# tangkk/audiomod

Hardware: AMD Instinct MI355X
Metric: Msamples/s (48 kHz stereo) phase-vocoder pitch-shift; x real-time per GPU (higher is better)
Workload: dtype f32; 1 GPU; configs[1]: normal_pitchshift +4 st, stereo 48 kHz, fft=2048, phase-locked; streams_per_gpu=128, channels=2, block=480, hop_in=203, slices_per_channel=14190, concurrent_stream_groups=1, parallelism=stream-sharded x1, no collective, rank_sync=none

## Files before the change

### audiomod_amd/csrc/pv_engine.cc

```cpp
#include <cstdio>
#include <cstdlib>
#include <cmath>
#include <algorithm>
#include <chrono>
#include <cstring>
#include <deque>
#include <memory>
#include <string>
#include <vector>

#include <hip/hip_runtime.h>

#include "audiomod_pv.h"
#include "pv_kernels.h"
#include "pv_wavefft.h"
#include "pv_plan.h"

namespace pv {

static thread_local std::string g_last_error;

static int hip_fail(hipError_t e, const char *what, int line) {
    char buf[512];
    snprintf(buf, sizeof buf, "%s failed at pv_engine.cc:%d: %s", what, line, hipGetErrorString(e));
// ... 208 lines not shown
    const ResTile *res_tiles;
    const uint2 *res_otab;
    int res_ntiles;
    hipStream_t res_stream;
    hipEvent_t ev_fused, ev_res, ev_ring_free;
    bool late_chain;
};

struct Core {
    Derived d;
    int device = 0, S = 0, C = 0, rows = 0;
    int Tc = 0, TR = 0, FR = 0, HP = 0, pkmax = 0, PKP = 0, lookback = 0;
    bool pipelined_planes = false;
    int ola_lds_floats = 0;
    int otab_off = 0, wacc_pitch = 0;
    DevTables tb{};
    DevBuf<int32_t> perm, iperm;
    DevBuf<float2> tw_fwd, tw_inv, st_fwd, st_inv;
    DevBuf<float4> twl_fwd, twl_inv;
    DevBuf<float> window, window_sh, sinc;
    DevBuf<float4> tab4;
    DevBuf<float> mag, phase, outphase, frames, rot;
    DevBuf<float> cmag, cphase;
    DevBuf<uint16_t> peaks;
    DevBuf<int32_t> npk, modes;
    DevBuf<PeakRec> recs;
    DevBuf<float> st_pp, st_po, st_rot;
    DevBuf<int32_t> st_kind;
    bool use_chain = false;
    bool chain_required = false;
    static constexpr int kChainMinRows = 192;
    bool fast_arith = false;
    bool fuse_phase = false;
    bool split_analysis = false;
    bool ahead = false;
    bool three_stage = false;
    int chain_AR = 0, chain_smask = 0, chain_waves = 0;
    int chain_max_adv = 0;
    DevBuf<float> st_acc, stream;
    mutable int acc_half = 0;
#ifdef PV_DIAG
    static bool debug_stale_acc() {
        static const bool on = [] {
            const char *e = getenv("AUDIOMOD_PV_DEBUG_STALE_ACC");
            return e && atoi(e) != 0;
        }();
        return on;
    }
#endif
    mutable hipError_t launch_err = hipSuccess;
    mutable int launch_err_line = 0;
    int take_launch_error() const {
        if (launch_err == hipSuccess) return PV_OK;
        const int rc = hip_fail(launch_err, "a launch / event call of Core::launch_chunk", launch_err_line);
        launch_err = hipSuccess;
        return rc;
    }
    void build_res_tiles(int64_t ka, int64_t kb, std::vector<ResTile> &tiles, std::vector<uint2> &otab) const;
    static bool chain_wanted() {
        const char *e = getenv("AUDIOMOD_PV_FUSED");
        if (e && atoi(e) == 0) return false;
        const char *sl = getenv("AUDIOMOD_PV_STREAM_LAUNCHES");
        return !(sl && strcmp(sl, "single") == 0);
    }
    bool wave_fft() const { return d.fft.nc == 256 || d.fft.nc == 512 || d.fft.nc == 1024 || d.fft.nc == 2048; }
    bool fast_chain() const { return use_chain && fast_capable(); }
// ... 134 lines not shown
    }
    TR = (nstreams > 0 && pipelined_planes) ? (ahead ? 3 : 2) * Tc + 1 : Tc + 1;
    FR = next_pow2_i(Tc + lookback + 1);

    std::vector<int32_t> ip(d.fft.nc);
    for (int j = 0; j < d.fft.nc; ++j) ip[d.fft.perm[j]] = j;
    if ((st = perm.upload(d.fft.perm)) != PV_OK) return st;
    if ((st = iperm.upload(ip)) != PV_OK) return st;
    auto up2 = [&](DevBuf<float2> &b, const std::vector<cpx> &v) -> int {
        std::vector<float2> t(v.size());
        for (size_t i = 0; i < v.size(); ++i) t[i] = make_float2(v[i].r, v[i].i);
        return b.upload(t);
    };
    if ((st = up2(tw_fwd, d.fft.tw_fwd)) != PV_OK) return st;
    if ((st = up2(tw_inv, d.fft.tw_inv)) != PV_OK) return st;
    if ((st = up2(st_fwd, d.fft.st_fwd)) != PV_OK) return st;
    if (wave_fft()) {
        auto lane_table = [&](const std::vector<cpx> &tw, DevBuf<float4> &dst) -> int {
            std::vector<cf> twc(tw.size());
            for (size_t i = 0; i < tw.size(); ++i) twc[i] = cf{tw[i].r, tw[i].i};
            const int entries = d.fft.nc == 256    ? wf_lane_table_entries<WF<256>>()
                                : d.fft.nc == 512  ? wf_lane_table_entries<WF<512>>()
                                : d.fft.nc == 1024 ? wf_lane_table_entries<WF<1024>>()
                                                   : wf_lane_table_entries<WF<2048>>();
            std::vector<cf> out(2 * (size_t)entries * 64);
            if (d.fft.nc == 256) wf_build_lane_table<WF<256>>(twc.data(), out.data());
            else if (d.fft.nc == 512) wf_build_lane_table<WF<512>>(twc.data(), out.data());
            else if (d.fft.nc == 1024) wf_build_lane_table<WF<1024>>(twc.data(), out.data());
            else wf_build_lane_table<WF<2048>>(twc.data(), out.data());
            std::vector<float4> o4((size_t)entries * 64);
            for (size_t i = 0; i < o4.size(); ++i) o4[i] = make_float4(out[2 * i].x, out[2 * i].y, out[2 * i + 1].x, out[2 * i + 1].y);
            return dst.upload(o4);
        };
        {
            const char *es = getenv("AUDIOMOD_PV_SPLIT_ANALYSIS");
            const char *sl = getenv("AUDIOMOD_PV_STREAM_LAUNCHES");
            split_analysis = d.fft.nc == 2048 && !(es && atoi(es) == 0) && !(sl && strcmp(sl, "single") == 0);
        }
        if (split_analysis) {
            std::vector<cf> twc(d.fft.tw_fwd.size());
            for (size_t i = 0; i < twc.size(); ++i) twc[i] = cf{d.fft.tw_fwd[i].r, d.fft.tw_fwd[i].i};
            const int entries = wf_lane_table_entries<WF2048S>();
            std::vector<cf> out(2 * (size_t)entries * WF2048S::LANES);
            wf_build_lane_table<WF2048S>(twc.data(), out.data());
            std::vector<float4> o4((size_t)entries * WF2048S::LANES);
            for (size_t i = 0; i < o4.size(); ++i) o4[i] = make_float4(out[2 * i].x, out[2 * i].y, out[2 * i + 1].x, out[2 * i + 1].y);
            if ((st = twl_fwd.upload(o4)) != PV_OK) return st;
        } else if ((st = lane_table(d.fft.tw_fwd, twl_fwd)) != PV_OK) return st;
        if ((st = lane_table(d.fft.tw_inv, twl_inv)) != PV_OK) return st;
    }
    if ((st = up2(st_inv, d.fft.st_inv)) != PV_OK) return st;
    if ((st = window.upload(d.window)) != PV_OK) return st;
    {
        const size_t pitch = (size_t)d.N + 8;
        std::vector<float> sh(4 * pitch, 0.f);
        for (int dd = 0; dd < 4; ++dd)
            for (int j = 0; j < d.N; ++j) sh[dd * pitch + j + dd] = d.window[j];
        if ((st = window_sh.upload(sh)) != PV_OK) return st;
    }
    if ((st = sinc.upload(d.sinc)) != PV_OK) return st;
    {
        std::vector<float4> t4;
        if (d.resample && d.interp) {
            t4.assign((size_t)d.oversample * (d.filt_len + 1), make_float4(0, 0, 0, 0));
            for (int off = 0; off < d.oversample; ++off)
                for (int j = 0; j < d.filt_len; ++j) {
// ... 231 lines not shown
    auto rec = [&](int i) {
        if (ev) HIPV(hipEventRecord(ev[i], st));
    };
    auto side_stream = [&](int k, auto &&launch_on) {
        if (defer_chain) return;
        if (part == 1) {
            HIPV(hipEventRecord(ev_match, st));
            HIPV(hipStreamWaitEvent(st_chain, ev_match, 0));
            if (ev) HIPV(hipEventRecord(ev[2 * k], st_chain));
            launch_on(st_chain);
            if (ev) HIPV(hipEventRecord(ev[2 * k + 1], st_chain));
            HIPV(hipEventRecord(ev_chain, st_chain));
        } else if (part == 2) {
            if (!only_resample) HIPV(hipStreamWaitEvent(st, ev_chain, 0));
        } else {
            rec(2 * k);
            launch_on(st);
            rec(2 * k + 1);
        }
    };
    AnalyzeArgs aa{};
    aa.tb = tb;
    aa.ia = ia;
    aa.hop = d.hop;
    const int s0 = (int)(t0 % TR);
    aa.t0 = t0;
    aa.s0 = s0;
    aa.Tn = Tn;
    aa.TR = TR;
    aa.rows = rows;
    aa.PKP = PKP;
    aa.find_peaks = cm == 1 ? 1 : 0;
    aa.split = split_analysis ? 1 : 0;
    aa.mag = mag.p;
    aa.phase = phase.p;
    aa.peaks = peaks.p;
    aa.npk = npk.p;
    const bool do_analysis = front && !only_chain && !no_analysis;
    if (do_analysis) rec(2 * PV_K_ANALYZE);
    if (single_launch) fused.aa = aa;
    else if (do_analysis) launch_analyze(aa, st); HIPV(hipGetLastError());
    if (do_analysis && d.vocoder && carrier) {
        AnalyzeArgs ca = aa;
        ca.ia = *carrier;
        ca.rows = 1;
        ca.find_peaks = 0;
        ca.mag = cmag.p;
        ca.phase = cphase.p;
        launch_analyze(ca, st); HIPV(hipGetLastError());
    }
    if (do_analysis) rec(2 * PV_K_ANALYZE + 1);
    if (only_analysis) return;

    if (cm == 1) {
        MatchArgs ma{};
        ma.N = d.N;
        ma.hs = d.hs;
        ma.HP = HP;
        ma.PKP = PKP;
        ma.C = C;
        ma.hop = d.hop;
        ma.TR = TR;
        ma.rows = rows;
        ma.Tn = Tn;
        ma.two_pi_hop = d.two_pi_hop;
        ma.t0 = t0;
// ... 2986 lines not shown
```

### audiomod_amd/csrc/pv_kernels.h

```cpp
#pragma once

#include <cstdint>

#include <hip/hip_runtime.h>

namespace pv {

constexpr int kFftThreads = 256;
constexpr int kTileOut = 256;
constexpr int kMaxTileFrames = 128;

struct DevTables {
    int N, hs, H, HP, nc, log2nc;
    int nstages;
    int radix[16], log2m[16], fstride[16];
    const int32_t *perm;
    const int32_t *iperm;
    const float2 *tw_fwd, *tw_inv, *st_fwd, *st_inv;
    const float4 *twl_fwd, *twl_inv;
    const float *window;
    const float *window_sh;
};

struct InAddr {
    const float *in;
    int64_t stride_s, stride_c;
    uint64_t mask;
    int64_t len;
};

enum : int { kModeInit = 0, kModeProp = 1, kModeLock = 2 };

struct AnalyzeArgs {
    DevTables tb;
    InAddr ia;
    int hop;
    int64_t t0;
    int s0;
    int Tn;
    int TR;
    int rows;
    int PKP;
    int find_peaks;
    int split;
    float *mag;
    float *phase;
    uint16_t *peaks;
    int32_t *npk;
};

struct PeakRec {
    float adv;
    float a2;
    float a1;
    uint32_t p1r1;
};

struct MatchArgs {
    int N, hs, HP, PKP, C, hop, TR, rows, Tn, s0;
    double two_pi_hop;
    int64_t t0;
    const int32_t *phase_inc;
    const float *phase;
    const uint16_t *peaks;
    const int32_t *npk;
    PeakRec *recs;
    int32_t *modes;
};

struct SeqArgs {
    int N, hs, HP, PKP, C, hop, TR, rows, Tn, s0;
    int high_prio;
    int narrow;
    double two_pi_hop;
    int64_t t0;
    const int32_t *phase_inc;
    const float *phase;
    const uint16_t *peaks;
    const int32_t *npk;
    const PeakRec *recs;
    const int32_t *modes;
// ... 254 lines not shown
```

### audiomod_amd/csrc/pv_kernels.hip

```cpp
#include "pv_kernels.h"
#include "pv_atan2f.h"
#include "pv_sincos.h"
#include "pv_wavefft.h"

#include <hip/hip_runtime.h>
#include <cstdlib>

namespace pv {

#ifdef PV_POISON
__device__ __forceinline__ void pv_poison_lds(char *base) {
    const uint32_t bytes = ((const __attribute__((address_space(4))) uint32_t *)__builtin_amdgcn_dispatch_ptr())[7];
    const int nt = blockDim.x * blockDim.y * blockDim.z, tid = threadIdx.x;
    for (uint32_t i = tid; i < bytes / 4; i += nt) reinterpret_cast<uint32_t *>(base)[i] = 0x7fc0dead;
    __syncthreads();
}
#define PV_POISON_LDS(base) pv_poison_lds(base)
#else
#define PV_POISON_LDS(base) ((void)0)
#endif

#define PV_PI 3.14159265358979323846

__device__ __forceinline__ float2 cmul(float2 a, float2 b) {
// ... 169 lines not shown

    const int lane = threadIdx.x & 63, wave = threadIdx.x >> 6, nw = nt >> 6;
    const int J = (hs + nt - 1) / nt;
    for (int j = 0; j < J; ++j) {
        const unsigned long long bm = __ballot(is_peak(smag, threadIdx.x + j * nt, hs));
        if (lane == 0) wcnt[j * nw + wave] = __popcll(bm);
    }
    __syncthreads();
    uint16_t *__restrict__ pk = a.peaks + plane * a.PKP;
    int running = 0, qi = 0;
    for (int j = 0; j < J; ++j) {
        const int mine = j * nw + wave;
        for (; qi < mine; ++qi) running += wcnt[qi];
        const int b = threadIdx.x + j * nt;
        const bool isp = is_peak(smag, b, hs);
        const unsigned long long bm = __ballot(isp);
        if (isp) pk[running + __popcll(bm & ((1ull << lane) - 1ull))] = (uint16_t)b;
    }
    if (threadIdx.x == 0) {
        int total = 0;
        for (int q = 0; q < J * nw; ++q) total += wcnt[q];
        a.npk[plane] = total;
    }
}

template <int WPB> __device__ __forceinline__ bool block_to_row_slice_w(int Tn, int rows, int &row, int &tl) {
    const int groups = (Tn + WPB - 1) / WPB;
    const int b = blockIdx.x, xcd = b & 7, q = b >> 3;
    row = xcd + 8 * (q / groups);
    tl = __builtin_amdgcn_readfirstlane(WPB * (q % groups) + (threadIdx.x >> 6));
    return row < rows && tl < Tn;
}

template <int NC, uint32_t ATAB>
__device__ __forceinline__ void analyze_wave_role(const AnalyzeArgs &a, const int row, const int tl, cf *lds) {
    typedef __attribute__((address_space(3))) uint32_t lds_u32;
    const unsigned char *atab = reinterpret_cast<const unsigned char *>((uintptr_t)ATAB);
    using W = WF<NC>;
    constexpr int N = 2 * NC, hs = NC, R = W::R;
    const int lane = threadIdx.x & 63;
    const uint32_t atab_word = pv_atan_blob_dev.w[lane];
    const DevTables &tb = a.tb;
    const int64_t t = a.t0 + tl;
    const int slot = ring_slot(a.s0, tl, a.TR);
    const int64_t a0 = t * (int64_t)a.hop;
    const float *__restrict__ in = a.ia.in + (int64_t)row * a.ia.stride_c;
    const float *__restrict__ w = tb.window;
    const cf *__restrict__ tw = reinterpret_cast<const cf *>(tb.tw_fwd);
    const cf *__restrict__ stw = reinterpret_cast<const cf *>(tb.st_fwd);
    const cf2 *__restrict__ twl = reinterpret_cast<const cf2 *>(tb.twl_fwd);

    WfTw<W> T0, T1, T2;
    wf_load_pass_tw<W, 0>(T0, lane, tw);
    cf v[R];
    {
        const int lp = wf_lane_part<W>(0, lane);
        const int lsrc = wf_src_of<W>(lp);
        const uint64_t m0 = (uint64_t)a0 & a.ia.mask;
        if (a0 + N + 4 <= a.ia.len && ((m0 + (uint64_t)(N + 3)) & a.ia.mask) == m0 + (uint64_t)(N + 3)) {
            const float *__restrict__ fp = in + m0;
            const uintptr_t fa = reinterpret_cast<uintptr_t>(fp);
            const int d = (int)((fa & 15u) >> 2);
            const float4 *__restrict__ xb = reinterpret_cast<const float4 *>(fa & ~(uintptr_t)15);
            const float4 *__restrict__ wb = reinterpret_cast<const float4 *>(tb.window_sh + (size_t)d * (N + 8));
            constexpr int Q = N / 256;
            float4 *stage4 = reinterpret_cast<float4 *>(lds);
            float4 xt = make_float4(0.f, 0.f, 0.f, 0.f), wt = xt;
            if (lane == 0) {
                xt = xb[64 * Q];
                wt = wb[64 * Q];
            }
            constexpr int QS = Q < 8 ? Q : 8;
#pragma unroll
            for (int q0 = 0; q0 < Q; q0 += QS) {
                float4 xq[QS], wq[QS];
#pragma unroll
                for (int q = 0; q < QS; ++q) {
                    xq[q] = xb[lane + 64 * (q0 + q)];
                    wq[q] = wb[lane + 64 * (q0 + q)];
                }
#pragma unroll
                for (int q = 0; q < QS; ++q)
                    stage4[lane + 64 * (q0 + q)] =
                        make_float4(xq[q].x * wq[q].x, xq[q].y * wq[q].y, xq[q].z * wq[q].z, xq[q].w * wq[q].w);
            }
            if (lane == 0) stage4[64 * Q] = make_float4(xt.x * wt.x, xt.y * wt.y, xt.z * wt.z, xt.w * wt.w);
            wave_sync();
            const float *stage = reinterpret_cast<const float *>(lds) + d;
            const int kl = (2 * lsrc + hs) & (N - 1);
#pragma unroll
            for (int r = 0; r < R; ++r) {
                const int kr = 2 * wf_src_of_const<W>(wf_reg_part<W>(0, r));
                const int k0 = kl ^ kr;
                v[r] = cf{stage[k0], stage[k0 + 1]};
            }
            wave_sync();
        } else {
#pragma unroll
            for (int r = 0; r < R; ++r) {
                const int src = lsrc | wf_src_of_const<W>(wf_reg_part<W>(0, r));
                const int k0 = (2 * src + hs) & (N - 1);
                const int64_t g0 = a0 + k0;
                const float x0 = g0 < a.ia.len ? in[(uint64_t)g0 & a.ia.mask] : 0.f;
                const float x1 = g0 + 1 < a.ia.len ? in[(uint64_t)(g0 + 1) & a.ia.mask] : 0.f;
                v[r] = cf{x0 * w[k0], x1 * w[k0 + 1]};
            }
        }
    }
    constexpr int J = NC / 128;
    const int lp0 = wf_lane_part<W>(0, lane), lp1 = wf_lane_part<W>(1, lane), lp2 = wf_lane_part<W>(2, lane);
    WfTwRaw<W, 1> raw1;
#if defined(PV_EXP_ANA) && (PV_EXP_ANA & 1)
#define PV_ANA_BFLY(x)
#else
#define PV_ANA_BFLY(x) x
#endif
#if defined(PV_EXP_ANA) && (PV_EXP_ANA & 2)
#define PV_ANA_XCHG(x)
#else
#define PV_ANA_XCHG(x) x
#endif
    wf_fetch_pass_tw<W, 1>(raw1, lane, twl);
    PV_ANA_BFLY((wf_apply_pass_stages<W, 0, false>(v, T0)));
    PV_ANA_XCHG((wf_store<W, 0>(lds, v, lp0)));
    wave_sync();
    PV_ANA_XCHG((wf_load<W, 1>(lds, v, lp1)));
    wf_unpack_pass_tw<W, 1>(T1, raw1);
    PV_ANA_BFLY((wf_apply_pass_stages<W, 1, false>(v, T1)));
    WfTwRaw<W, 2> raw2;
    wf_fetch_pass_tw<W, 2>(raw2, lane, twl);
    PV_ANA_XCHG((wf_store<W, 1>(lds, v, lp1)));
    wave_sync();
    PV_ANA_XCHG((wf_load<W, 2>(lds, v, lp2)));
    wf_unpack_pass_tw<W, 2>(T2, raw2);
    PV_ANA_BFLY((wf_apply_pass_stages<W, 2, false>(v, T2)));
    if constexpr (W::NPASS == 4) {
        const int lp3 = wf_lane_part<W>(3, lane);
        WfTwRaw<W, 3> raw3;
        wf_fetch_pass_tw<W, 3>(raw3, lane, twl);
        PV_ANA_XCHG((wf_store<W, 2>(lds, v, lp2)));
        wave_sync();
// ... 35 lines not shown
    if (lane == 0) {
        const cf fpk = lds[W::pad(NC / 2)];
        const cf fpnk = cf{fpk.x, -fpk.y};
        const cf f1k = wf_add(fpk, fpnk);
        const cf f2k = wf_sub(fpk, fpnk);
        const cf tq = wf_cmul(f2k, swmid);
        xmid = cf{(f1k.x - tq.x) * 0.5f, (tq.y - f1k.y) * 0.5f};
    }
    wave_sync();
#pragma unroll
    for (int j = 0; j < J; ++j) {
        const int k = lane + 64 * j;
        if (j == 0 && lane == 0) {
            lds[0] = xlo[0];
            lds[NC] = xhi[0];
        } else {
            lds[k] = xlo[j];
            lds[NC - k] = xhi[j];
        }
    }
    if (lane == 0) lds[NC / 2] = xmid;
    wave_sync();
    float *smag = reinterpret_cast<float *>(lds);
    *(lds_u32 *)(uintptr_t)(ATAB + 4u * (uint32_t)lane) = atab_word;
    float edge_mag = 0.f, edge_ph = 0.f;
    if (lane < 2) {
        const cf e = lds[lane == 0 ? 0 : NC];
        edge_mag = sqrtf(e.x * e.x + 0.f * 0.f);
        edge_ph = pv_u2f((uint32_t)((int32_t)pv_f2u(e.x) >> 31) & pv_f2u(3.1415927410e+00f));
    }
    wave_sync();
    if (lane == 0) lds[0] = cf{1.f, 1.f};
    wave_sync();
#pragma nounroll
    for (int q = 0; q < NC / 256; ++q) {
        const int i4 = 4 * (lane + 64 * q);
        const float4 c01 = *reinterpret_cast<const float4 *>(lds + i4);
        const float4 c23 = *reinterpret_cast<const float4 *>(lds + i4 + 2);
        float4 m4, p4;
        const float a0 = c01.x * c01.x + c01.y * c01.y, a1 = c01.z * c01.z + c01.w * c01.w;
        const float a2 = c23.x * c23.x + c23.y * c23.y, a3 = c23.z * c23.z + c23.w * c23.w;
        const float mx = __builtin_fmaxf(__builtin_fmaxf(pv_max3_abs(c01.x, c01.y, c01.z), pv_max3_abs(c01.w, c23.x, c23.y)),
                                         __builtin_fmaxf(__builtin_fabsf(c23.z), __builtin_fabsf(c23.w)));
        const float mn = __builtin_fminf(__builtin_fminf(pv_min3_abs(c01.x, c01.y, c01.z), pv_min3_abs(c01.w, c23.x, c23.y)),
                                         __builtin_fminf(__builtin_fabsf(c23.z), __builtin_fabsf(c23.w)));
        const bool in_range = mx < 0x1p63f && mn >= 0x1p-48f;
#if defined(PV_EXP_ANA) && (PV_EXP_ANA & 4)
        if (true) {
            m4 = make_float4(a0, a1, a2, a3);
            p4 = make_float4(c01.y + mx, c01.w + mn, c23.y, c23.w);
        } else
#endif
        if (__builtin_amdgcn_ballot_w64(!in_range) == 0) {
            m4 = make_float4(pv_sqrt_safe(a0), pv_sqrt_safe(a1), pv_sqrt_safe(a2), pv_sqrt_safe(a3));
            p4.x = pv_atan2f_fd_tab<true>(c01.y, c01.x, atab);
            p4.y = pv_atan2f_fd_tab<true>(c01.w, c01.z, atab);
            p4.z = pv_atan2f_fd_tab<true>(c23.y, c23.x, atab);
            p4.w = pv_atan2f_fd_tab<true>(c23.w, c23.z, atab);
        } else {
            m4 = make_float4(sqrtf(a0), sqrtf(a1), sqrtf(a2), sqrtf(a3));
            p4.x = pv_atan2f_fd_tab<false>(c01.y, c01.x, atab);
            p4.y = pv_atan2f_fd_tab<false>(c01.w, c01.z, atab);
            p4.z = pv_atan2f_fd_tab<false>(c23.y, c23.x, atab);
            p4.w = pv_atan2f_fd_tab<false>(c23.w, c23.z, atab);
        }
        if (q == 0 && lane == 0) p4.x = edge_ph, m4.x = edge_mag;
#if !(defined(PV_EXP_ANA) && (PV_EXP_ANA & 8))
        *reinterpret_cast<float4 *>(ph + i4) = p4;
        *reinterpret_cast<float4 *>(mag + i4) = m4;
#else
        if (p4.x == 12345.678f) *reinterpret_cast<float4 *>(ph + i4) = p4;
#endif
        *reinterpret_cast<float4 *>(smag + i4) = m4;
    }
    if (lane == 1) {
        ph[NC] = edge_ph;
        mag[NC] = edge_mag;
        smag[NC] = edge_mag;
    }
    wave_sync();
#if defined(PV_EXP_ANA) && (PV_EXP_ANA & 16)
    if (lane == 0) a.npk[plane] = 100;
    return;
#endif
    if (!a.find_peaks) return;
    uint16_t *slist = reinterpret_cast<uint16_t *>(smag + NC + 4);
    int running = 0;
    const float inf = __builtin_inff();
#pragma unroll
    for (int q = 0; q < NC / 256; ++q) {
        const int i4 = 4 * (lane + 64 * q);
        const float4 m = *reinterpret_cast<const float4 *>(smag + i4);
        float2 lo = *reinterpret_cast<const float2 *>(smag + (q == 0 && lane == 0 ? 0 : i4 - 2));
        float2 hi = *reinterpret_cast<const float2 *>(smag + i4 + 4);
        if (q == 0 && lane == 0) lo = make_float2(inf, inf);
        if (q == NC / 256 - 1 && lane == 63) hi = make_float2(inf, inf);
        const float in01 = __builtin_fmaxf(m.x, m.y), in12 = __builtin_fmaxf(m.y, m.z), in23 = __builtin_fmaxf(m.z, m.w);
        const bool f0 = m.x > __builtin_fmaxf(__builtin_fmaxf(lo.x, lo.y), in12);
        const bool f1 = m.y > __builtin_fmaxf(__builtin_fmaxf(lo.y, m.x), in23);
        const bool f2 = m.z > __builtin_fmaxf(in01, __builtin_fmaxf(m.w, hi.x));
        const bool f3 = m.w > __builtin_fmaxf(in12, __builtin_fmaxf(hi.x, hi.y));
        const bool any = f0 || f1 || f2 || f3, two = f0 && f3;
        const unsigned long long ma = __ballot(any), mb = __ballot(two);
        const int pos = running + (int)__builtin_amdgcn_mbcnt_hi((unsigned)(ma >> 32), __builtin_amdgcn_mbcnt_lo((unsigned)ma, 0u)) +
                        (int)__builtin_amdgcn_mbcnt_hi((unsigned)(mb >> 32), __builtin_amdgcn_mbcnt_lo((unsigned)mb, 0u));
        if (any) slist[pos] = (uint16_t)(i4 + (f0 ? 0 : f1 ? 1 : f2 ? 2 : 3));
        if (two) slist[pos + 1] = (uint16_t)(i4 + 3);
        running += __popcll(ma) + __popcll(mb);
    }
    if (lane == 0) {
        a.npk[plane] = running;
        if (running & 1) slist[running] = 0;
    }
    wave_sync();
    uint32_t *__restrict__ pk32 = reinterpret_cast<uint32_t *>(a.peaks + plane * a.PKP);
    const uint32_t *slist32 = reinterpret_cast<const uint32_t *>(slist);
    for (int i = lane; 2 * i < running; i += 64) pk32[i] = slist32[i];
}

__device__ __forceinline__ void lds_barrier() { asm volatile("s_waitcnt lgkmcnt(0)\n\ts_barrier" ::: "memory"); }

template <class W, uint32_t ATAB>
__device__ __forceinline__ void analyze_split_role(const AnalyzeArgs &a, const int row, const int tl, cf *lds) {
    typedef __attribute__((address_space(3))) uint32_t lds_u32;
    const unsigned char *atab = reinterpret_cast<const unsigned char *>((uintptr_t)ATAB);
    constexpr int NC = W::N_C, N = 2 * NC, hs = NC, R = W::R, LN = W::LANES;
    const int tid = threadIdx.x, lane = tid & 63;
    const int wv = __builtin_amdgcn_readfirstlane(tid >> 6);
    const uint32_t atab_word = pv_atan_blob_dev.w[lane];
    const DevTables &tb = a.tb;
    const int64_t t = a.t0 + tl;
    const int slot = ring_slot(a.s0, tl, a.TR);
    const int64_t a0 = t * (int64_t)a.hop;
    const float *__restrict__ in = a.ia.in + (int64_t)row * a.ia.stride_c;
    const float *__restrict__ w = tb.window;
    const cf *__restrict__ tw = reinterpret_cast<const cf *>(tb.tw_fwd);
    const cf *__restrict__ stw = reinterpret_cast<const cf *>(tb.st_fwd);
    const cf2 *__restrict__ twl = reinterpret_cast<const cf2 *>(tb.twl_fwd);

    WfTw<W> T0, T1, T2;
    wf_load_pass_tw<W, 0>(T0, tid, tw);
    cf v[R];
    {
        const int lp = wf_lane_part<W>(0, tid);
        const int lsrc = wf_src_of<W>(lp);
        const uint64_t m0 = (uint64_t)a0 & a.ia.mask;
        if (a0 + N + 4 <= a.ia.len && ((m0 + (uint64_t)(N + 3)) & a.ia.mask) == m0 + (uint64_t)(N + 3)) {
            const float *__restrict__ fp = in + m0;
            const uintptr_t fa = reinterpret_cast<uintptr_t>(fp);
            const int d = (int)((fa & 15u) >> 2);
// ... 192 lines not shown
        const int pos = running + (wv ? c0 : 0) + pre[q];
        const int i4 = 4 * (tid + LN * q);
        if (fl[q] & 4) slist[pos] = (uint16_t)(i4 + (fl[q] & 3));
        if (fl[q] & 8) slist[pos + 1] = (uint16_t)(i4 + 3);
        running += c0 + c1;
    }
    if (tid == 0) {
        a.npk[plane] = running;
        if (running & 1) slist[running] = 0;
    }
    lds_barrier();
    uint32_t *__restrict__ pk32 = reinterpret_cast<uint32_t *>(a.peaks + plane * a.PKP);
    const uint32_t *slist32 = reinterpret_cast<const uint32_t *>(slist);
    for (int i = tid; 2 * i < running; i += LN) pk32[i] = slist32[i];
}

__global__ __launch_bounds__(128) void pv_analyze_split_kernel(const AnalyzeArgs a) {
    extern __shared__ __attribute__((aligned(16))) char smem_raw[];
    PV_POISON_LDS(reinterpret_cast<char *>(smem_raw));
    int row, tl;
    if (!block_to_row_slice(a.Tn, a.rows, row, tl)) return;
    analyze_split_role<WF2048S, WF2048S::LDS_CF * sizeof(cf)>(a, row, tl, reinterpret_cast<cf *>(smem_raw));
}

template <int NC, int WPB> __global__ __launch_bounds__(64 * WPB) void pv_analyze_wave_kernel(const AnalyzeArgs a) {
    extern __shared__ __attribute__((aligned(16))) char smem_raw[];
    PV_POISON_LDS(reinterpret_cast<char *>(smem_raw));
    cf *lds = reinterpret_cast<cf *>(smem_raw) + (threadIdx.x >> 6) * WF<NC>::LDS_CF;
    int row, tl;
    if (!block_to_row_slice_w<WPB>(a.Tn, a.rows, row, tl)) return;
    analyze_wave_role<NC, WPB * WF<NC>::LDS_CF * sizeof(cf)>(a, row, tl, lds);
}

template <typename K> static void allow_big_lds_dev(K kernel, unsigned long long &done_mask) {
    int dev = 0;
    (void)hipGetDevice(&dev);
    const unsigned long long bit = 1ull << (dev & 63);
    if (__atomic_load_n(&done_mask, __ATOMIC_ACQUIRE) & bit) return;
    (void)hipFuncSetAttribute(reinterpret_cast<const void *>(kernel), hipFuncAttributeMaxDynamicSharedMemorySize,
                              160 * 1024 - 512);
    __atomic_fetch_or(&done_mask, bit, __ATOMIC_RELEASE);
}

void launch_analyze(const AnalyzeArgs &a, hipStream_t st) {
    if (a.tb.nc == 512 || a.tb.nc == 256) {
        constexpr int WPB = 1;
        const int grid = 8 * ((a.rows + 7) / 8) * ((a.Tn + WPB - 1) / WPB);
        if (a.tb.nc == 512)
            hipLaunchKernelGGL((pv_analyze_wave_kernel<512, WPB>), dim3(grid), dim3(64 * WPB),
                               WPB * WF<512>::LDS_CF * sizeof(cf) + 4 * PV_ATAN_BLOB_WORDS, st, a);
        else
            hipLaunchKernelGGL((pv_analyze_wave_kernel<256, WPB>), dim3(grid), dim3(64 * WPB),
                               WPB * WF<256>::LDS_CF * sizeof(cf) + 4 * PV_ATAN_BLOB_WORDS, st, a);
        return;
    }
    if (a.tb.nc == 1024 || a.tb.nc == 2048) {
        if (a.tb.nc == 1024) {
            constexpr int WPB = 1;
            const int grid = 8 * ((a.rows + 7) / 8) * ((a.Tn + WPB - 1) / WPB);
            hipLaunchKernelGGL((pv_analyze_wave_kernel<1024, WPB>), dim3(grid), dim3(64 * WPB),
                               WPB * WF<1024>::LDS_CF * sizeof(cf) + 4 * PV_ATAN_BLOB_WORDS, st, a);
        } else {
            if (a.split) {
                const int grid = 8 * ((a.rows + 7) / 8) * a.Tn;
                hipLaunchKernelGGL(pv_analyze_split_kernel, dim3(grid), dim3(WF2048S::LANES),
                                   WF2048S::LDS_CF * sizeof(cf) + 4 * PV_ATAN_BLOB_WORDS + 64, st, a);
                return;
            }
            constexpr int WPB = 1;
            const int grid = 8 * ((a.rows + 7) / 8) * ((a.Tn + WPB - 1) / WPB);
            static unsigned long long big = 0;
            allow_big_lds_dev(pv_analyze_wave_kernel<2048, WPB>, big);
            hipLaunchKernelGGL((pv_analyze_wave_kernel<2048, WPB>), dim3(grid), dim3(64 * WPB),
                               WPB * WF<2048>::LDS_CF * sizeof(cf) + 4 * PV_ATAN_BLOB_WORDS, st, a);
        }
        return;
    }
// ... 3735 lines not shown
```

Measured before the change: 17750 Msamples/s.

## Add multi-frame walk analysis kernel that prefetches the next frame's input during FFT

Adds a walk analysis kernel for nc 256/512/1024 in which each 64-lane wave processes F consecutive frames of one row. While the current frame's FFT and polar/peak stages run, it issues the next frame's input and window vector loads, aiming to hide global-load latency behind compute. The existing per-frame analysis is refactored into reusable load, stage and transform helpers with before-polar and before-peaks hooks. It is chosen by default when rows times frame-groups reaches a threshold, or forced through an environment variable. The cost is fewer, longer-lived waves, which lowers parallelism and raises register pressure from holding the prefetched loads.

```diff
diff --git a/audiomod_amd/csrc/pv_engine.cc b/audiomod_amd/csrc/pv_engine.cc
--- a/audiomod_amd/csrc/pv_engine.cc
+++ b/audiomod_amd/csrc/pv_engine.cc
@@ -264,6 +264,7 @@
     static constexpr int kChainMinRows = 192;
     bool fast_arith = false;
     bool fuse_phase = false;
+    int analysis_walk = -1;
     bool split_analysis = false;
     bool ahead = false;
     bool three_stage = false;
@@ -464,6 +465,11 @@
             for (size_t i = 0; i < o4.size(); ++i) o4[i] = make_float4(out[2 * i].x, out[2 * i].y, out[2 * i + 1].x, out[2 * i + 1].y);
             return dst.upload(o4);
         };
+        {
+            const char *ew = getenv("AUDIOMOD_PV_ANALYSIS_WALK");
+            const int v = ew ? atoi(ew) : -1;
+            analysis_walk = (v == 0 || v == 2 || v == 4 || v == 8) ? v : -1;
+        }
         {
             const char *es = getenv("AUDIOMOD_PV_SPLIT_ANALYSIS");
             const char *sl = getenv("AUDIOMOD_PV_STREAM_LAUNCHES");
@@ -761,6 +767,7 @@
     aa.PKP = PKP;
     aa.find_peaks = cm == 1 ? 1 : 0;
     aa.split = split_analysis ? 1 : 0;
+    aa.walk = analysis_walk;
     aa.mag = mag.p;
     aa.phase = phase.p;
     aa.peaks = peaks.p;
diff --git a/audiomod_amd/csrc/pv_kernels.h b/audiomod_amd/csrc/pv_kernels.h
--- a/audiomod_amd/csrc/pv_kernels.h
+++ b/audiomod_amd/csrc/pv_kernels.h
@@ -47,6 +47,7 @@
     float *phase;
     uint16_t *peaks;
     int32_t *npk;
+    int walk;
 };
 
 struct PeakRec {
diff --git a/audiomod_amd/csrc/pv_kernels.hip b/audiomod_amd/csrc/pv_kernels.hip
--- a/audiomod_amd/csrc/pv_kernels.hip
+++ b/audiomod_amd/csrc/pv_kernels.hip
@@ -225,81 +225,144 @@
     return row < rows && tl < Tn;
 }
 
-template <int NC, uint32_t ATAB>
-__device__ __forceinline__ void analyze_wave_role(const AnalyzeArgs &a, const int row, const int tl, cf *lds) {
+
+typedef float ana_v4f __attribute__((ext_vector_type(4)));
+typedef const __attribute__((address_space(1))) ana_v4f ana_gv4f;
+__device__ __forceinline__ ana_v4f ana_ld4(const ana_gv4f *p) { return *p; }
+struct AnaFrame {
+    int64_t a0;
+    const float *in;
+    int fast;
+    int d;
+    const ana_gv4f *xb, *wb;
+};
+template <int NC> __device__ __forceinline__ AnaFrame ana_frame(const AnalyzeArgs &a, const int row, const int tl) {
+    constexpr int N = 2 * NC;
+    AnaFrame f;
+    const int64_t t = a.t0 + tl;
+    f.a0 = t * (int64_t)a.hop;
+    f.in = a.ia.in + (int64_t)row * a.ia.stride_c;
+    const uint64_t m0 = (uint64_t)f.a0 & a.ia.mask;
+    f.fast = f.a0 + N + 4 <= a.ia.len && ((m0 + (uint64_t)(N + 3)) & a.ia.mask) == m0 + (uint64_t)(N + 3);
+    const uintptr_t fa = reinterpret_cast<uintptr_t>(f.in + m0);
+    f.d = (int)((fa & 15u) >> 2);
+    f.xb = reinterpret_cast<const ana_gv4f *>(fa & ~(uintptr_t)15);
+    f.wb = reinterpret_cast<const ana_gv4f *>(reinterpret_cast<uintptr_t>(a.tb.window_sh + (size_t)f.d * (N + 8)));
+    return f;
+}
+
+template <int NC> struct AnaLoads {
+    static constexpr int Q = 2 * NC / 256, QS = Q < 8 ? Q : 8;
+    ana_v4f xq[QS], wq[QS], xt, wt;
+};
+typedef const __attribute__((address_space(4))) ana_v4f ana_cv4f;
+__device__ __forceinline__ ana_v4f ana_ld4_uniform(const ana_gv4f *p) {
+    return *reinterpret_cast<ana_cv4f *>(reinterpret_cast<uintptr_t>(p));
+}
+template <int NC, int Q0, bool WIN = true, bool SCAL = false>
+__device__ __forceinline__ void ana_issue_loads(const AnaFrame &f, const int lane, AnaLoads<NC> &L) {
+    using A = AnaLoads<NC>;
+    if constexpr (Q0 == 0 && SCAL) {
+        L.xt = ana_ld4_uniform(f.xb + 64 * A::Q);
+        if constexpr (WIN) L.wt = ana_ld4_uniform(f.wb + 64 * A::Q);
+    } else if constexpr (Q0 == 0) {
+        L.xt = ana_v4f(0.f);
+        if constexpr (WIN) L.wt = L.xt;
+        if (lane == 0) {
+            L.xt = ana_ld4(f.xb + 64 * A::Q);
+            if constexpr (WIN) L.wt = ana_ld4(f.wb + 64 * A::Q);
+        }
+    }
+#pragma unroll
+    for (int q = 0; q < A::QS; ++q) {
+        L.xq[q] = ana_ld4(f.xb + lane + 64 * (Q0 + q));
+        if constexpr (WIN) L.wq[q] = ana_ld4(f.wb + lane + 64 * (Q0 + q));
+    }
+}
+template <int NC, int Q0, bool SCAL = false>
+__device__ __forceinline__ void ana_issue_window(const AnaFrame &f, const int lane, AnaLoads<NC> &L) {
+    using A = AnaLoads<NC>;
+    if constexpr (Q0 == 0 && SCAL) {
+        L.wt = ana_ld4_uniform(f.wb + 64 * A::Q);
+    } else if constexpr (Q0 == 0) {
+        L.wt = ana_v4f(0.f);
+        if (lane == 0) L.wt = ana_ld4(f.wb + 64 * A::Q);
+    }
+#pragma unroll
+    for (int q = 0; q < A::QS; ++q) L.wq[q] = ana_ld4(f.wb + lane + 64 * (Q0 + q));
+}
+__device__ __forceinline__ void ana_touch(ana_v4f &x) { asm volatile("" : "+v"(x)); }
+template <int NC, int Q0> __device__ __forceinline__ void ana_mul_stage(const AnaLoads<NC> &L, const int lane, cf *lds) {
+    using A = AnaLoads<NC>;
+    ana_v4f *stage4 = reinterpret_cast<ana_v4f *>(lds);
+#pragma unroll
+    for (int q = 0; q < A::QS; ++q) stage4[lane + 64 * (Q0 + q)] = L.xq[q] * L.wq[q];
+}
+template <int NC>
+__device__ __forceinline__ void ana_read_pass0(const AnaFrame &f, const AnaLoads<NC> &L, const int lane, cf *lds,
+                                               cf (&v)[WF<NC>::R]) {
+    using W = WF<NC>;
+    constexpr int N = 2 * NC, hs = NC, R = W::R;
+    ana_v4f *stage4 = reinterpret_cast<ana_v4f *>(lds);
+    if (lane == 0) stage4[64 * AnaLoads<NC>::Q] = L.xt * L.wt;
+    wave_sync();
+    const int lsrc = wf_src_of<W>(wf_lane_part<W>(0, lane));
+    const float *stage = reinterpret_cast<const float *>(lds) + f.d;
+    const int kl = (2 * lsrc + hs) & (N - 1);
+#pragma unroll
+    for (int r = 0; r < R; ++r) {
+        const int kr = 2 * wf_src_of_const<W>(wf_reg_part<W>(0, r));
+        const int k0 = kl ^ kr;
+        v[r] = cf{stage[k0], stage[k0 + 1]};
+    }
+    wave_sync();
+}
+template <int NC>
+__device__ __forceinline__ void ana_edge_frame(const AnalyzeArgs &a, const AnaFrame &f, const int lane, cf (&v)[WF<NC>::R]) {
+    using W = WF<NC>;
+    constexpr int N = 2 * NC, hs = NC, R = W::R;
+    const float *__restrict__ in = f.in;
+    const float *__restrict__ w = a.tb.window;
+    const int lsrc = wf_src_of<W>(wf_lane_part<W>(0, lane));
+#pragma unroll
+    for (int r = 0; r < R; ++r) {
+        const int src = lsrc | wf_src_of_const<W>(wf_reg_part<W>(0, r));
+        const int k0 = (2 * src + hs) & (N - 1);
+        const int64_t g0 = f.a0 + k0;
+        const float x0 = g0 < a.ia.len ? in[(uint64_t)g0 & a.ia.mask] : 0.f;
+        const float x1 = g0 + 1 < a.ia.len ? in[(uint64_t)(g0 + 1) & a.ia.mask] : 0.f;
+        v[r] = cf{x0 * w[k0], x1 * w[k0 + 1]};
+    }
+}
+template <int NC>
+__device__ __forceinline__ void ana_load_frame(const AnalyzeArgs &a, const AnaFrame &f, const int lane, cf *lds, cf (&v)[WF<NC>::R]) {
+    if (f.fast) {
+        AnaLoads<NC> L;
+        ana_issue_loads<NC, 0>(f, lane, L);
+        ana_mul_stage<NC, 0>(L, lane, lds);
+        if constexpr (AnaLoads<NC>::Q > 8) {
+            static_assert(AnaLoads<NC>::Q <= 16, "two batches of eight pieces at the most");
+            ana_issue_loads<NC, 8>(f, lane, L);
+            ana_mul_stage<NC, 8>(L, lane, lds);
+        }
+        ana_read_pass0<NC>(f, L, lane, lds, v);
+    } else {
+        ana_edge_frame<NC>(a, f, lane, v);
+    }
+}
+
+template <int NC, uint32_t ATAB, bool WALK, class BeforePolar, class BeforePeaks>
+__device__ __forceinline__ void ana_transform(const AnalyzeArgs &a, const int row, const int tl, const int lane, cf *lds,
+                                              cf (&v)[WF<NC>::R], const WfTw<WF<NC>> &T0, const uint32_t atab_word,
+                                              BeforePolar &&before_polar, BeforePeaks &&before_peaks) {
     typedef __attribute__((address_space(3))) uint32_t lds_u32;
     const unsigned char *atab = reinterpret_cast<const unsigned char *>((uintptr_t)ATAB);
     using W = WF<NC>;
-    constexpr int N = 2 * NC, hs = NC, R = W::R;
-    const int lane = threadIdx.x & 63;
-    const uint32_t atab_word = pv_atan_blob_dev.w[lane];
     const DevTables &tb = a.tb;
-    const int64_t t = a.t0 + tl;
     const int slot = ring_slot(a.s0, tl, a.TR);
-    const int64_t a0 = t * (int64_t)a.hop;
-    const float *__restrict__ in = a.ia.in + (int64_t)row * a.ia.stride_c;
-    const float *__restrict__ w = tb.window;
-    const cf *__restrict__ tw = reinterpret_cast<const cf *>(tb.tw_fwd);
     const cf *__restrict__ stw = reinterpret_cast<const cf *>(tb.st_fwd);
     const cf2 *__restrict__ twl = reinterpret_cast<const cf2 *>(tb.twl_fwd);
-
-    WfTw<W> T0, T1, T2;
-    wf_load_pass_tw<W, 0>(T0, lane, tw);
-    cf v[R];
-    {
-        const int lp = wf_lane_part<W>(0, lane);
-        const int lsrc = wf_src_of<W>(lp);
-        const uint64_t m0 = (uint64_t)a0 & a.ia.mask;
-        if (a0 + N + 4 <= a.ia.len && ((m0 + (uint64_t)(N + 3)) & a.ia.mask) == m0 + (uint64_t)(N + 3)) {
-            const float *__restrict__ fp = in + m0;
-            const uintptr_t fa = reinterpret_cast<uintptr_t>(fp);
-            const int d = (int)((fa & 15u) >> 2);
-            const float4 *__restrict__ xb = reinterpret_cast<const float4 *>(fa & ~(uintptr_t)15);
-            const float4 *__restrict__ wb = reinterpret_cast<const float4 *>(tb.window_sh + (size_t)d * (N + 8));
-            constexpr int Q = N / 256;
-            float4 *stage4 = reinterpret_cast<float4 *>(lds);
-            float4 xt = make_float4(0.f, 0.f, 0.f, 0.f), wt = xt;
-            if (lane == 0) {
-                xt = xb[64 * Q];
-                wt = wb[64 * Q];
-            }
-            constexpr int QS = Q < 8 ? Q : 8;
-#pragma unroll
-            for (int q0 = 0; q0 < Q; q0 += QS) {
-                float4 xq[QS], wq[QS];
-#pragma unroll
-                for (int q = 0; q < QS; ++q) {
-                    xq[q] = xb[lane + 64 * (q0 + q)];
-                    wq[q] = wb[lane + 64 * (q0 + q)];
-                }
-#pragma unroll
-                for (int q = 0; q < QS; ++q)
-                    stage4[lane + 64 * (q0 + q)] =
-                        make_float4(xq[q].x * wq[q].x, xq[q].y * wq[q].y, xq[q].z * wq[q].z, xq[q].w * wq[q].w);
-            }
-            if (lane == 0) stage4[64 * Q] = make_float4(xt.x * wt.x, xt.y * wt.y, xt.z * wt.z, xt.w * wt.w);
-            wave_sync();
-            const float *stage = reinterpret_cast<const float *>(lds) + d;
-            const int kl = (2 * lsrc + hs) & (N - 1);
-#pragma unroll
-            for (int r = 0; r < R; ++r) {
-                const int kr = 2 * wf_src_of_const<W>(wf_reg_part<W>(0, r));
-                const int k0 = kl ^ kr;
-                v[r] = cf{stage[k0], stage[k0 + 1]};
-            }
-            wave_sync();
-        } else {
-#pragma unroll
-            for (int r = 0; r < R; ++r) {
-                const int src = lsrc | wf_src_of_const<W>(wf_reg_part<W>(0, r));
-                const int k0 = (2 * src + hs) & (N - 1);
-                const int64_t g0 = a0 + k0;
-                const float x0 = g0 < a.ia.len ? in[(uint64_t)g0 & a.ia.mask] : 0.f;
-                const float x1 = g0 + 1 < a.ia.len ? in[(uint64_t)(g0 + 1) & a.ia.mask] : 0.f;
-                v[r] = cf{x0 * w[k0], x1 * w[k0 + 1]};
-            }
-        }
-    }
+    WfTw<W> T1, T2;
     constexpr int J = NC / 128;
     const int lp0 = wf_lane_part<W>(0, lane), lp1 = wf_lane_part<W>(1, lane), lp2 = wf_lane_part<W>(2, lane);
     WfTwRaw<W, 1> raw1;
@@ -401,6 +464,7 @@
     wave_sync();
     if (lane == 0) lds[0] = cf{1.f, 1.f};
     wave_sync();
+    before_polar();
 #pragma nounroll
     for (int q = 0; q < NC / 256; ++q) {
         const int i4 = 4 * (lane + 64 * q);
@@ -448,43 +512,66 @@
         smag[NC] = edge_mag;
     }
     wave_sync();
+    before_peaks();
 #if defined(PV_EXP_ANA) && (PV_EXP_ANA & 16)
     if (lane == 0) a.npk[plane] = 100;
     return;
 #endif
-    if (!a.find_peaks) return;
-    uint16_t *slist = reinterpret_cast<uint16_t *>(smag + NC + 4);
-    int running = 0;
-    const float inf = __builtin_inff();
-#pragma unroll
-    for (int q = 0; q < NC / 256; ++q) {
-        const int i4 = 4 * (lane + 64 * q);
-        const float4 m = *reinterpret_cast<const float4 *>(smag + i4);
-        float2 lo = *reinterpret_cast<const float2 *>(smag + (q == 0 && lane == 0 ? 0 : i4 - 2));
-        float2 hi = *reinterpret_cast<const float2 *>(smag + i4 + 4);
-        if (q == 0 && lane == 0) lo = make_float2(inf, inf);
-        if (q == NC / 256 - 1 && lane == 63) hi = make_float2(inf, inf);
-        const float in01 = __builtin_fmaxf(m.x, m.y), in12 = __builtin_fmaxf(m.y, m.z), in23 = __builtin_fmaxf(m.z, m.w);
-        const bool f0 = m.x > __builtin_fmaxf(__builtin_fmaxf(lo.x, lo.y), in12);
-        const bool f1 = m.y > __builtin_fmaxf(__builtin_fmaxf(lo.y, m.x), in23);
-        const bool f2 = m.z > __builtin_fmaxf(in01, __builtin_fmaxf(m.w, hi.x));
-        const bool f3 = m.w > __builtin_fmaxf(in12, __builtin_fmaxf(hi.x, hi.y));
-        const bool any = f0 || f1 || f2 || f3, two = f0 && f3;
-        const unsigned long long ma = __ballot(any), mb = __ballot(two);
-        const int pos = running + (int)__builtin_amdgcn_mbcnt_hi((unsigned)(ma >> 32), __builtin_amdgcn_mbcnt_lo((unsigned)ma, 0u)) +
-                        (int)__builtin_amdgcn_mbcnt_hi((unsigned)(mb >> 32), __builtin_amdgcn_mbcnt_lo((unsigned)mb, 0u));
-        if (any) slist[pos] = (uint16_t)(i4 + (f0 ? 0 : f1 ? 1 : f2 ? 2 : 3));
-        if (two) slist[pos + 1] = (uint16_t)(i4 + 3);
-        running += __popcll(ma) + __popcll(mb);
-    }
-    if (lane == 0) {
-        a.npk[plane] = running;
-        if (running & 1) slist[running] = 0;
-    }
-    wave_sync();
-    uint32_t *__restrict__ pk32 = reinterpret_cast<uint32_t *>(a.peaks + plane * a.PKP);
-    const uint32_t *slist32 = reinterpret_cast<const uint32_t *>(slist);
-    for (int i = lane; 2 * i < running; i += 64) pk32[i] = slist32[i];
+    if (a.find_peaks) {
+        uint16_t *slist = reinterpret_cast<uint16_t *>(smag + NC + 4);
+        int running = 0;
+        const float inf = __builtin_inff();
+#pragma unroll
+        for (int q = 0; q < NC / 256; ++q) {
+            const int i4 = 4 * (lane + 64 * q);
+            const float4 m = *reinterpret_cast<const float4 *>(smag + i4);
+            float2 lo = *reinterpret_cast<const float2 *>(smag + (q == 0 && lane == 0 ? 0 : i4 - 2));
+            float2 hi = *reinterpret_cast<const float2 *>(smag + i4 + 4);
+            if (q == 0 && lane == 0) lo = make_float2(inf, inf);
+            if (q == NC / 256 - 1 && lane == 63) hi = make_float2(inf, inf);
+            const float in01 = __builtin_fmaxf(m.x, m.y), in12 = __builtin_fmaxf(m.y, m.z), in23 = __builtin_fmaxf(m.z, m.w);
+            const bool f0 = m.x > __builtin_fmaxf(__builtin_fmaxf(lo.x, lo.y), in12);
+            const bool f1 = m.y > __builtin_fmaxf(__builtin_fmaxf(lo.y, m.x), in23);
+            const bool f2 = m.z > __builtin_fmaxf(in01, __builtin_fmaxf(m.w, hi.x));
+            const bool f3 = m.w > __builtin_fmaxf(in12, __builtin_fmaxf(hi.x, hi.y));
+            const bool any = f0 || f1 || f2 || f3, two = f0 && f3;
+            const unsigned long long ma = __ballot(any), mb = __ballot(two);
+            const int pos = running + (int)__builtin_amdgcn_mbcnt_hi((unsigned)(ma >> 32), __builtin_amdgcn_mbcnt_lo((unsigned)ma, 0u)) +
+                            (int)__builtin_amdgcn_mbcnt_hi((unsigned)(mb >> 32), __builtin_amdgcn_mbcnt_lo((unsigned)mb, 0u));
+            if (any) slist[pos] = (uint16_t)(i4 + (f0 ? 0 : f1 ? 1 : f2 ? 2 : 3));
+            if (two) slist[pos + 1] = (uint16_t)(i4 + 3);
+            running += __popcll(ma) + __popcll(mb);
+        }
+        if (lane == 0) {
+            a.npk[plane] = running;
+            if (running & 1) slist[running] = 0;
+        }
+        wave_sync();
+        uint32_t *__restrict__ pk32 = reinterpret_cast<uint32_t *>(a.peaks + plane * a.PKP);
+        const uint32_t *slist32 = reinterpret_cast<const uint32_t *>(slist);
+        if constexpr (WALK) {
+            constexpr int NW = (NC / 3 + 2 + 1) / 2;
+#pragma unroll
+            for (int j = 0; j < (NW + 63) / 64; ++j) {
+                const int i = lane + 64 * j;
+                if (2 * i < running) pk32[i] = slist32[i];
+            }
+        } else {
+            for (int i = lane; 2 * i < running; i += 64) pk32[i] = slist32[i];
+        }
+    }
+}
+
+template <int NC, uint32_t ATAB>
+__device__ __forceinline__ void analyze_wave_role(const AnalyzeArgs &a, const int row, const int tl, cf *lds) {
+    using W = WF<NC>;
+    const int lane = threadIdx.x & 63;
+    const uint32_t atab_word = pv_atan_blob_dev.w[lane];
+    WfTw<W> T0;
+    wf_load_pass_tw<W, 0>(T0, lane, reinterpret_cast<const cf *>(a.tb.tw_fwd));
+    cf v[W::R];
+    ana_load_frame<NC>(a, ana_frame<NC>(a, row, tl), lane, lds, v);
+    ana_transform<NC, ATAB, false>(a, row, tl, lane, lds, v, T0, atab_word, [] {}, [] {});
 }
 
 __device__ __forceinline__ void lds_barrier() { asm volatile("s_waitcnt lgkmcnt(0)\n\ts_barrier" ::: "memory"); }
@@ -743,6 +830,90 @@
     analyze_wave_role<NC, WPB * WF<NC>::LDS_CF * sizeof(cf)>(a, row, tl, lds);
 }
 
+#ifndef PV_ANA_WALK_PREFETCH
+#define PV_ANA_WALK_PREFETCH 3
+#endif
+#ifndef PV_ANA_WALK_DEFAULT_F
+#define PV_ANA_WALK_DEFAULT_F 4
+#endif
+template <int NC, int F> __global__ __launch_bounds__(64) void pv_analyze_walk_kernel(const AnalyzeArgs a) {
+    extern __shared__ __attribute__((aligned(16))) char smem_raw[];
+    PV_POISON_LDS(reinterpret_cast<char *>(smem_raw));
+    using W = WF<NC>;
+    static_assert(AnaLoads<NC>::Q <= 8, "one batch of pieces per frame");
+    constexpr int kPre = PV_ANA_WALK_PREFETCH;
+    cf *lds = reinterpret_cast<cf *>(smem_raw);
+    const int groups = (a.Tn + F - 1) / F;
+    const int b = blockIdx.x, xcd = b & 7, q = b >> 3;
+    const int row = xcd + 8 * (q / groups);
+    if (row >= a.rows) return;
+    const int tl0 = __builtin_amdgcn_readfirstlane(F * (q % groups));
+    const int n = __builtin_amdgcn_readfirstlane(a.Tn - tl0 < F ? a.Tn - tl0 : F);
+    const uint32_t atab_word = pv_atan_blob_dev.w[threadIdx.x];
+    const cf *__restrict__ tw = reinterpret_cast<const cf *>(a.tb.tw_fwd);
+    AnaLoads<NC> L;
+    AnaFrame f = ana_frame<NC>(a, row, tl0);
+    bool have = false;
+    for (int i = 0; i < n; ++i) {
+        const int tl = tl0 + i;
+        int lane = threadIdx.x;
+        asm volatile("" : "+v"(lane));
+        WfTw<W> T0;
+        wf_load_pass_tw<W, 0>(T0, lane, tw);
+        cf v[W::R];
+        if (f.fast) {
+            if (!have) {
+                ana_issue_loads<NC, 0, true, true>(f, lane, L);
+#pragma unroll
+                for (int j = 0; j < AnaLoads<NC>::QS; ++j) ana_touch(L.xq[j]), ana_touch(L.wq[j]);
+            } else if constexpr (kPre >= 4) {
+                ana_issue_window<NC, 0, true>(f, lane, L);
+            }
+            ana_mul_stage<NC, 0>(L, lane, lds);
+            ana_read_pass0<NC>(f, L, lane, lds, v);
+        } else {
+            ana_edge_frame<NC>(a, f, lane, v);
+        }
+        AnaFrame fn = f;
+        bool pf = false;
+        if (i + 1 < n) {
+            fn = ana_frame<NC>(a, row, tl + 1);
+            pf = fn.fast != 0;
+        }
+        auto issue = [&](const bool x, const bool w) {
+            const ana_v4f z = ana_v4f(0.f);
+            if (pf) {
+                if (x && w) ana_issue_loads<NC, 0, true, true>(fn, lane, L);
+                else if (x) ana_issue_loads<NC, 0, false, true>(fn, lane, L);
+                else ana_issue_window<NC, 0, true>(fn, lane, L);
+            } else {
+#pragma unroll
+                for (int j = 0; j < AnaLoads<NC>::QS; ++j) {
+                    if (x) L.xq[j] = z;
+                    if (w) L.wq[j] = z;
+                }
+                if (x) L.xt = z;
+                if (w) L.wt = z;
+            }
+        };
+        ana_transform<NC, W::LDS_CF * sizeof(cf), true>(
+            a, row, tl, lane, lds, v, T0, atab_word,
+            [&] {
+                if constexpr (kPre == 3) issue(true, true);
+                if constexpr (kPre == 2 || kPre == 5) issue(true, false);
+            },
+            [&] {
+                if constexpr (kPre == 2) issue(false, true);
+                if constexpr (kPre == 1) issue(true, true);
+                if constexpr (kPre == 4) issue(true, false);
+            });
+        f = fn;
+        have = pf;
+        wave_sync();
+        PV_POISON_LDS(reinterpret_cast<char *>(smem_raw));
+    }
+}
+
 template <typename K> static void allow_big_lds_dev(K kernel, unsigned long long &done_mask) {
     int dev = 0;
     (void)hipGetDevice(&dev);
@@ -753,7 +924,32 @@
     __atomic_fetch_or(&done_mask, bit, __ATOMIC_RELEASE);
 }
 
+constexpr int kWalkDefaultF = PV_ANA_WALK_DEFAULT_F, kWalkMinFills = 3;
+static int analyze_walk_frames(const AnalyzeArgs &a) {
+    if (a.tb.nc != 1024 && a.tb.nc != 512 && a.tb.nc != 256) return 0;
+    if (a.walk == 0 || a.walk == 2 || a.walk == 4 || a.walk == 8) return a.walk;
+    if (kWalkDefaultF == 0) return 0;
+    const int64_t waves = (int64_t)a.rows * ((a.Tn + kWalkDefaultF - 1) / kWalkDefaultF);
+    return waves >= (int64_t)kWalkMinFills * 4096 ? kWalkDefaultF : 0;
+}
+template <int NC, int F> static void launch_analyze_walk(const AnalyzeArgs &a, hipStream_t st) {
+    const int grid = 8 * ((a.rows + 7) / 8) * ((a.Tn + F - 1) / F);
+    hipLaunchKernelGGL((pv_analyze_walk_kernel<NC, F>), dim3(grid), dim3(64), WF<NC>::LDS_CF * sizeof(cf) + 4 * PV_ATAN_BLOB_WORDS,
+                       st, a);
+}
+template <int NC> static void launch_analyze_walk(const AnalyzeArgs &a, int F, hipStream_t st) {
+    if (F == 2) launch_analyze_walk<NC, 2>(a, st);
+    else if (F == 4) launch_analyze_walk<NC, 4>(a, st);
+    else launch_analyze_walk<NC, 8>(a, st);
+}
+
 void launch_analyze(const AnalyzeArgs &a, hipStream_t st) {
+    if (const int F = analyze_walk_frames(a)) {
+        if (a.tb.nc == 1024) launch_analyze_walk<1024>(a, F, st);
+        else if (a.tb.nc == 512) launch_analyze_walk<512>(a, F, st);
+        else launch_analyze_walk<256>(a, F, st);
+        return;
+    }
     if (a.tb.nc == 512 || a.tb.nc == 256) {
         constexpr int WPB = 1;
         const int grid = 8 * ((a.rows + 7) / 8) * ((a.Tn + WPB - 1) / WPB);
```

Result: slower. 17520 Msamples/s (-1.2%).
